# gaozhihan/PreDiff

Hardware: AMD Instinct MI355X
Metric: denoising_steps_per_sec (higher is better)
Workload: dtype bf16; 1 GPU; SEVIR-LR 7->6 x128x128 (latent 13x16x16, C 256/512, depth [4,4], axial), DDIM-50 eta=0, no knowledge alignment (BASELINE.json configs[1]); trajectories_per_gpu=64, global_trajectories=64, sampler=ddim50, hip_graph=True, lanes=2, trajectories_per_launch=32, parallelism=ensemble-shard x1

## Files before the change

### prediff_amd/csrc/conv3d_halo.hip

```cpp
#include <algorithm>
#include "common.h"
#include "igemm_epilogue.h"

namespace PD_NS {

#define BLDS16(rsrc, ldsptr, voff, soff) \
  __builtin_amdgcn_raw_ptr_buffer_load_lds((rsrc), (__attribute__((address_space(3))) void*)(ldsptr), 16, (voff), (soff), 0, 0)
#define PD_OOB 0xffffff00u
#define VMCNT(n) asm volatile("s_waitcnt vmcnt(" #n ")" ::: "memory")
#define PHASE_SYNC()                   \
  __builtin_amdgcn_sched_barrier(0);   \
  __builtin_amdgcn_s_barrier();        \
  __builtin_amdgcn_sched_barrier(0)

namespace {
constexpr int FW = 16;
constexpr int HW = FW + 2;
constexpr int HROWS = HW * HW;
constexpr int PLROWS = 336;
constexpr int PLANE = PLROWS * 16;
constexpr int HALO = 8 * PLANE;
constexpr int NPIECE = HALO / 1024;
constexpr int WHT = 128 * 128;
constexpr int WBUF = 2 * WHT;
// ... 88 lines not shown
  const bool dense = (p.debug_flags & 8) != 0;
  const int kt_lo = (dense || L) ? 0 : max(0, 1 - ot), kt_hi = (dense || L) ? 2 : min(2, p.Ti - ot);
  const int ngroups = (p.debug_flags & 1) ? 0 : kchunks * (kt_hi - kt_lo + 1);
  const uint32_t frame_b = (uint32_t)(L ? FW1 * FW1 : FW * FW) * (uint32_t)p.lda * 2u;
  uint32_t vm_all = 0;
  if constexpr (L == 1) {
    int o = (4 * tm) % p.To;
    for (int f = 0; f < 4; ++f) {
      if (4 * tm + f < p.B * p.To)
        for (int kt = 0; kt < 3; ++kt)
          if ((unsigned)(o - 1 + kt) < (unsigned)p.Ti) vm_all |= 1u << (4 * kt + f);
      if (++o == p.To) o = 0;
    }
  }
  const uint32_t w_tap_b = (uint32_t)p.w_tap_stride * 2u;

  int h_c = 0, h_kt = kt_lo, w_c = 0, w_kt = kt_lo;
  uint32_t w_off = (uint32_t)(kt_lo * 9) * w_tap_b;
  int h_soff = 0;
  uint32_t h_mask = 0, h_back = 0;
  char* const h_dst = smem + wave * 1024;
  char* const w_dst = smem + W_OFF + wave * 1024;
  auto next_halo = [&]() {
    if constexpr (L == 0) {
      const int it = ot - 1 + h_kt;
      const bool ok = (unsigned)it < (unsigned)p.Ti;
      h_soff = __builtin_amdgcn_readfirstlane(ok ? (int)((uint32_t)(tm - 1 + h_kt) * frame_b + (uint32_t)h_c * 128u) : 0);
      h_mask = ok ? 0u : PD_OOB;
    } else {
      const int fin = 4 * tm - 1 + h_kt, fb = max(fin, 0);
      h_soff = __builtin_amdgcn_readfirstlane((int)((uint32_t)fb * frame_b + (uint32_t)h_c * 128u));
      h_back = (uint32_t)(fb - fin) * frame_b;
      h_mask = (vm_all >> (4 * h_kt)) & 15u;
    }
    if (++h_kt > kt_hi) { h_kt = kt_lo; ++h_c; }
  };
  auto issue_h = [&](int n, int buf) {
    uint32_t v;
    if constexpr (L == 0) v = hoff[n] | h_mask;
    else v = ((h_mask >> (hoff[n] & 7u)) & 1u) ? (hoff[n] & ~7u) - h_back : PD_OOB;
    BLDS16(rA, h_dst + buf * HALO + n * 8192, v, h_soff);
  };
  auto next_w_group = [&]() {
    if (++w_kt > kt_hi) { w_kt = kt_lo; ++w_c; }
    w_off = (uint32_t)(w_kt * 9) * w_tap_b + (uint32_t)w_c * 128u;
  };
  auto issue_w = [&](int buf) {
    const int so = __builtin_amdgcn_readfirstlane((int)w_off);
    char* dst = w_dst + buf * WBUF;
    BLDS16(rW, dst, woff[0][0], so);
    BLDS16(rW, dst + 64 * 128, woff[0][1], so);
    BLDS16(rW, dst + WHT, woff[1][0], so);
    BLDS16(rW, dst + WHT + 64 * 128, woff[1][1], so);
    w_off += w_tap_b;
  };

  f32x4 acc[8][4];
#pragma unroll
  for (int i = 0; i < 8; ++i)
#pragma unroll
    for (int j = 0; j < 4; ++j)
#pragma unroll
      for (int r = 0; r < 4; ++r) acc[i][j][r] = 0.f;

  const int l16 = lane & 15, lg = lane >> 4;
  const int swz = (l16 >> 1) & 7;
  const int a_rd = (L ? wr * WROW1 + (l16 >> 3) * FPAIR1 + (l16 & 7) : wr * (8 * HW) + l16) * 16 + lg * PLANE;
  const int b_rd = W_OFF + (wc >> 1) * WHT + ((wc & 1) * 64 + l16) * 128;

  if (ngroups > 0) {
    next_halo();
    if (wave < NEXTRA) issue_h(5, 0);
#pragma unroll
    for (int n = 0; n < 5; ++n) issue_h(n, 0);
    issue_w(0);
    issue_w(1);
    VMCNT(4);
  }
  __builtin_amdgcn_s_barrier();
  if (wr == 1) __builtin_amdgcn_s_barrier();
  __builtin_amdgcn_sched_barrier(0);

  FragH a[4], b0[2], b1[2];
#define LOAD_B(f, base) \
  (f).v[0] = *(const op8*)((base) + ((lg ^ swz) * 16)); (f).v[1] = *(const op8*)((base) + (((4 + lg) ^ swz) * 16))
#define LOAD_A(f, base) \
  (f).v[0] = *(const op8*)(base); (f).v[1] = *(const op8*)((base) + 4 * PLANE)
#define QUAD16(R0, C0, bfrag)                                                                               \
  _Pragma("unroll") for (int ks = 0; ks < 2; ++ks)                                                          \
    _Pragma("unroll") for (int i = 0; i < 4; ++i)                                                           \
      _Pragma("unroll") for (int c = 0; c < 2; ++c)                                                         \
        acc[(R0) + i][(C0) + c] = mfma_16x16x32(a[i].v[ks], bfrag[c].v[ks], acc[(R0) + i][(C0) + c]);

  int wcur = 0;
  auto group = [&](auto has_next_t, int g) {
    constexpr bool has_next = decltype(has_next_t)::value;
    const int hnxt = (g & 1) ^ 1;
    const char* sA = smem + (g & 1) * HALO + a_rd;
    if (has_next) next_halo();
#pragma unroll
    for (int j = 0; j < 9; ++j) {
      const int shift = ((j / 3) * PITCH + (j % 3)) * 16;
      const char* sB = smem + wcur * WBUF + b_rd;
#pragma unroll
      for (int c = 0; c < 2; ++c) { LOAD_B(b0[c], sB + c * (16 * 128)); }
#pragma unroll
      for (int i = 0; i < 4; ++i) { LOAD_A(a[i], sA + shift + i * (PITCH * 16)); }
#pragma unroll
      for (int c = 0; c < 2; ++c) { LOAD_B(b1[c], sB + (2 + c) * (16 * 128)); }
      if (j >= 1 && j <= 5 && has_next) {
        if (j == 1 && wave < NEXTRA) issue_h(5, hnxt);
        issue_h(j - 1, hnxt);
      }
      PHASE_SYNC();
      __builtin_amdgcn_s_setprio(1);
      QUAD16(0, 0, b0)
      QUAD16(0, 2, b1)
      __builtin_amdgcn_s_setprio(0);
      PHASE_SYNC();
#pragma unroll
      for (int i = 0; i < 4; ++i) { LOAD_A(a[i], sA + shift + (4 + i) * (PITCH * 16)); }
      if (j <= 6 || has_next) {
        if (j == 7) next_w_group();
        issue_w(wcur);
        if (j >= 1 && j <= 5 && has_next) {
          VMCNT(5);
        } else {
          VMCNT(4);
        }
      } else {
        VMCNT(0);
      }
      PHASE_SYNC();
      __builtin_amdgcn_s_setprio(1);
      QUAD16(4, 2, b1)
      QUAD16(4, 0, b0)
      __builtin_amdgcn_s_setprio(0);
      PHASE_SYNC();
      wcur ^= 1;
    }
  };
  for (int g = 0; g + 1 < ngroups; ++g) group(std::true_type{}, g);
  if (ngroups > 0) group(std::false_type{}, ngroups - 1);
#undef QUAD16
#undef LOAD_A
#undef LOAD_B
  if (wr == 0) __builtin_amdgcn_s_barrier();
  if (p.debug_flags & 2) return;

  float* sC = (float*)smem + wave * (128 * 32);
  const int m_base = m0 + wr * 128;
  const int m_end = min(p.M, m_base + 128);
  const int c_row = L ? (lg >> 1) * 64 + (lg & 1) * 4 : 4 * lg;
#pragma unroll
  for (int js = 0; js < 2; ++js) {
    __syncthreads();
#pragma unroll
    for (int i = 0; i < 8; ++i)
#pragma unroll
      for (int c = 0; c < 2; ++c)
#pragma unroll
        for (int r = 0; r < 4; ++r) sC[(c_row + i * (L ? 8 : 16) + r) * 32 + c * 16 + l16] = acc[i][js * 2 + c][r];
    __syncthreads();
    igemm_epilogue<128, 32>(p, sC, lane, m_base, m_end, n0 + wc * 64 + js * 32, 0);
  }
#endif
}

bool pd_conv3d_halo_supported(const pd_igemm_args& a, int kind, int level) {
  if (kind != 2 || a.split || a.fp8 || a.w_fold > 0 || a.nbatch > 1) return false;
  if (a.KT != 3 || a.KH != 3 || a.KW != 3 || a.pt != 1 || a.ph != 1 || a.pw != 1) return false;
  if (a.st != 1 || a.sh != 1 || a.sw != 1 || a.ut != 1 || a.uh != 1 || a.uw != 1 || a.vT > 0 || a.vH > 0 || a.vW > 0) return false;
  const int fw = level ? FW1 : FW;
  return a.Hi == fw && a.Wi == fw && a.Ho == fw && a.Wo == fw && a.Ti == a.To;
}

template <int L>
static int launch_halo(const pd_igemm_args& a, hipStream_t s) {
  constexpr int LDS = Lay<L>::LDS;
  static bool attr_set_dev[PD_MAX_DEVICES];
  bool& attr_set = attr_set_dev[pd_cur_device()];
  if (!attr_set) {
    hipError_t e = hipFuncSetAttribute((const void*)conv3d_halo_kernel<L>, hipFuncAttributeMaxDynamicSharedMemorySize, LDS);
    if (e != hipSuccess) {
      pd_set_error("pd_igemm: hipFuncSetAttribute(%d) failed: %s", LDS, hipGetErrorString(e));
      return PD_ERR_LAUNCH;
    }
    attr_set = true;
  }
  const int tiles = ((a.M + 255) / 256) * ((a.N + 255) / 256);
  hipLaunchKernelGGL(conv3d_halo_kernel<L>, dim3(tiles, 1, 1), dim3(512), LDS, s, a);
  PD_CHECK_LAUNCH();
  return PD_OK;
}

int pd_conv3d_halo_launch(const pd_igemm_args& a, int level, hipStream_t s) { return level ? launch_halo<1>(a, s) : launch_halo<0>(a, s); }

}
```

### prediff_amd/csrc/igemm.hip

```cpp
#include <type_traits>
#include "common.h"
#include "igemm_epilogue.h"

namespace PD_NS {

__device__ __attribute__((aligned(64))) uint32_t g_pd_zero_page[32];

#ifndef PD_BIG_TILE_DEFAULT
#define PD_BIG_TILE_DEFAULT 1
#endif

#define BLDS16(rsrc, ldsptr, voff, soff) \
  __builtin_amdgcn_raw_ptr_buffer_load_lds((rsrc), (__attribute__((address_space(3))) void*)(ldsptr), 16, (voff), (soff), 0, 0)
#define PD_OOB 0xffffff00u

template <int N>
__device__ __forceinline__ void wait_vmcnt() {
  asm volatile("s_waitcnt vmcnt(%0)" ::"n"(N) : "memory");
}

template <int BM, int BN, int BK, int NS, bool SPLIT, int KIND, int OCC = 2, int ESLAB = 1>
__global__ void __launch_bounds__(256, OCC) igemm_kernel(const pd_igemm_args p) {
#if defined(__HIP_DEVICE_COMPILE__)
  constexpr int ROWB = BK * 2;
// ... 8 lines not shown
  constexpr int KSUB = BK / 32;
  extern __shared__ __attribute__((aligned(16))) char smem[];

  const int tid = threadIdx.x;
  const int lane = tid & 63;
  const int wave = __builtin_amdgcn_readfirstlane(tid >> 6);

  const int tiles_n = (p.N + BN - 1) / BN;
  const int tiles_m = (p.M + BM - 1) / BM;
  const int nt = tiles_m * tiles_n;
  int t;
  {
    const int bid = blockIdx.x, xcd = bid & 7, q = nt >> 3, r = nt & 7;
    t = (xcd < r ? xcd * (q + 1) : r * (q + 1) + (xcd - r) * q) + (bid >> 3);
  }
  const int m0 = (t / tiles_n) * BM;
  const int n0 = (t % tiles_n) * BN;
  const int bz = blockIdx.z;

  const auto rA = __builtin_amdgcn_make_buffer_rsrc((void*)(p.A + (int64_t)bz * p.a_batch_stride), 0, p.a_bytes, 0x00020000);
  const auto rW = __builtin_amdgcn_make_buffer_rsrc((void*)(p.W + (int64_t)bz * p.w_batch_stride), 0, p.w_bytes, 0x00020000);
  const auto rAlo = __builtin_amdgcn_make_buffer_rsrc((void*)((SPLIT ? p.A_lo : p.A) + (int64_t)bz * p.a_batch_stride), 0, p.a_bytes, 0x00020000);
  const auto rWlo = __builtin_amdgcn_make_buffer_rsrc((void*)((SPLIT ? p.W_lo : p.W) + (int64_t)bz * p.w_batch_stride), 0, p.w_bytes, 0x00020000);

  const int srow = tid / CPR;
  const int spos = tid % CPR;
  const int schunk = (CPR == 8) ? (spos ^ ((srow >> 1) & 7)) : (spos ^ ((srow >> 2) & 3));
  int vt0[AI], vh0[AI], vw0[AI];
  uint32_t abase[AI];
  uint32_t aoff[AI];
#pragma unroll
  for (int i = 0; i < AI; ++i) {
    const int m = m0 + i * RPI + srow;
    if (KIND == 0) {
      aoff[i] = m < p.M ? ((uint32_t)m * (uint32_t)p.lda + schunk * 8) * 2u : PD_OOB;
    } else {
      const int hw_o = p.Ho * p.Wo, thw_o = p.To * hw_o;
      const bool ok = m < p.M;
      const int mm = ok ? m : 0;
      const int b = mm / thw_o, r1 = mm - b * thw_o;
      const int ot = r1 / hw_o, r2 = r1 - ot * hw_o;
      const int oh = r2 / p.Wo, ow = r2 - oh * p.Wo;
      vt0[i] = ok ? ot * p.st - p.pt : -(1 << 20);
      vh0[i] = oh * p.sh - p.ph;
      vw0[i] = ow * p.sw - p.pw;
      abase[i] = (uint32_t)b * (uint32_t)(p.Ti * p.Hi * p.Wi);
    }
  }
  uint32_t woff[BI];
#pragma unroll
  for (int i = 0; i < BI; ++i) {
    const int n = n0 + i * RPI + srow;
    woff[i] = n < p.N ? ((uint32_t)n * (uint32_t)p.ldw + schunk * 8) * 2u : PD_OOB;
  }
  const int kchunks = p.Cin / BK;
  const int nk = (p.debug_flags & 1) ? 0 : p.taps * kchunks;
  const int vT = p.vT > 0 ? p.vT : p.Ti * p.ut, vH = p.vH > 0 ? p.vH : p.Hi * p.uh, vW = p.vW > 0 ? p.vW : p.Wi * p.uw;
  const int khw = p.KH * p.KW;

  auto set_tap = [&](int tap) {
    if (p.w_fold > 0 && tap >= p.w_fold) tap -= p.w_fold;
    const int kt = tap / khw, r = tap - kt * khw;
    const int kh = r / p.KW, kw = r - kh * p.KW;
#pragma unroll
    for (int i = 0; i < AI; ++i) {
      const int vt = vt0[i] + kt, vh = vh0[i] + kh, vw = vw0[i] + kw;
      const bool ok = (unsigned)vt < (unsigned)vT && (unsigned)vh < (unsigned)vH && (unsigned)vw < (unsigned)vW;
      const int it = p.ut == 2 ? vt >> 1 : vt, ih = p.uh == 2 ? vh >> 1 : vh, iw = p.uw == 2 ? vw >> 1 : vw;
      aoff[i] = ok ? ((abase[i] + (uint32_t)((it * p.Hi + ih) * p.Wi + iw)) * (uint32_t)p.lda + schunk * 8) * 2u : PD_OOB;
    }
  };

  auto issue = [&](int stage, int ks) {
    const int tap = ks / kchunks, kc = ks - tap * kchunks;
    if (KIND != 0 && kc == 0) set_tap(tap);
    char* sbase = smem + stage * STAGE;
    const int ka = kc * (BK * 2);
    const int kw = (int)(((int64_t)tap * p.w_tap_stride + kc * BK) * 2);
#pragma unroll
    for (int i = 0; i < AI; ++i) {
      char* dst = sbase + (i * 256 + wave * 64) * 16;
      BLDS16(rA, dst, aoff[i], ka);
      if (SPLIT) BLDS16(rAlo, dst + A_TILE, aoff[i], ka);
    }
#pragma unroll
    for (int i = 0; i < BI; ++i) {
      char* dst = sbase + A_TILE * NP + (i * 256 + wave * 64) * 16;
      BLDS16(rW, dst, woff[i], kw);
      if (SPLIT) BLDS16(rWlo, dst + B_TILE, woff[i], kw);
    }
  };

  constexpr int TM16 = BM / 32, TN16 = BN / 32;
  f32x4 acc[TM16][TN16];
#pragma unroll
  for (int i = 0; i < TM16; ++i)
#pragma unroll
    for (int j = 0; j < TN16; ++j)
#pragma unroll
      for (int r = 0; r < 4; ++r) acc[i][j][r] = 0.f;

  const int wr = wave >> 1, wc = wave & 1;
  const int l16 = lane & 15, lg = lane >> 4;
  const int swz = (CPR == 8) ? ((l16 >> 1) & 7) : ((l16 >> 2) & 3);
  const int a_row_b = (wr * (BM / 2) + l16) * ROWB;
  const int b_row_b = (wc * (BN / 2) + l16) * ROWB;

  constexpr int D = NS - 1;
#pragma unroll
  for (int s0 = 0; s0 < D; ++s0)
    if (s0 < nk) issue(s0, s0);
  int stage = 0;
  for (int ks = 0; ks < nk; ++ks) {
    const int younger = min(D - 1, nk - ks - 1);
    if (D >= 3 && younger == 2) wait_vmcnt<2 * LPS>();
    else if (D >= 2 && younger == 1) wait_vmcnt<LPS>();
    else wait_vmcnt<0>();
    __builtin_amdgcn_s_barrier();
    if (ks + D < nk) issue((stage + D) % NS, ks + D);
    const char* sA = smem + stage * STAGE;
    const char* sB = sA + A_TILE * NP;
#pragma unroll
    for (int kk = 0; kk < KSUB; ++kk) {
      const int pos = ((kk * 4 + lg) ^ swz) * 16;
      op8 a[TM16], b[TN16], al[TM16], bl[TN16];
#pragma unroll
      for (int i = 0; i < TM16; ++i) {
        a[i] = *(const op8*)(sA + a_row_b + i * 16 * ROWB + pos);
        if (SPLIT) al[i] = *(const op8*)(sA + A_TILE + a_row_b + i * 16 * ROWB + pos);
      }
#pragma unroll
      for (int j = 0; j < TN16; ++j) {
        b[j] = *(const op8*)(sB + b_row_b + j * 16 * ROWB + pos);
        if (SPLIT) bl[j] = *(const op8*)(sB + B_TILE + b_row_b + j * 16 * ROWB + pos);
      }
#pragma unroll
      for (int i = 0; i < TM16; ++i)
#pragma unroll
        for (int j = 0; j < TN16; ++j) {
          if (SPLIT) {
            acc[i][j] = mfma_16x16x32(al[i], b[j], acc[i][j]);
            acc[i][j] = mfma_16x16x32(a[i], bl[j], acc[i][j]);
          }
          acc[i][j] = mfma_16x16x32(a[i], b[j], acc[i][j]);
        }
    }
    stage = stage + 1 == NS ? 0 : stage + 1;
  }

  constexpr int WM = BM / 2, WN = BN / 2;
  constexpr int WNS = WN / ESLAB;
  constexpr int TNS = TN16 / ESLAB;
  float* sC = (float*)smem + wave * (WM * WNS);
#pragma unroll
  for (int js = 0; js < ESLAB; ++js) {
    __syncthreads();
#pragma unroll
    for (int i = 0; i < TM16; ++i)
#pragma unroll
      for (int j = 0; j < TNS; ++j)
#pragma unroll
        for (int r = 0; r < 4; ++r)
          sC[(i * 16 + 4 * lg + r) * WNS + j * 16 + l16] = acc[i][js * TNS + j][r];
    __syncthreads();
    igemm_epilogue<WM, WNS>(p, sC, lane, m0 + wr * WM, p.M, n0 + wc * WN + js * WNS, bz);
  }
#endif
}

template <int BM, int BN, int BK, int NS, bool SPLIT, int KIND, int OCC = 2, int ESLAB = 1>
static int launch_igemm(const pd_igemm_args& a, hipStream_t s) {
  constexpr int stage = (BM + BN) * BK * 2 * (SPLIT ? 2 : 1);
  constexpr int epi = 4 * (BM / 2) * (BN / 2) * 4 / ESLAB;
  constexpr int lds = NS * stage > epi ? NS * stage : epi;
  static bool attr_set_dev[PD_MAX_DEVICES];
  bool& attr_set = attr_set_dev[pd_cur_device()];
  if (!attr_set) {
    hipError_t e = hipFuncSetAttribute((const void*)igemm_kernel<BM, BN, BK, NS, SPLIT, KIND, OCC, ESLAB>,
                                       hipFuncAttributeMaxDynamicSharedMemorySize, lds);
    if (e != hipSuccess) {
      pd_set_error("pd_igemm: hipFuncSetAttribute(%d) failed: %s", lds, hipGetErrorString(e));
      return PD_ERR_LAUNCH;
    }
    attr_set = true;
  }
  const int tiles = ((a.M + BM - 1) / BM) * ((a.N + BN - 1) / BN);
  dim3 grid(tiles, 1, a.nbatch > 0 ? a.nbatch : 1);
  hipLaunchKernelGGL((igemm_kernel<BM, BN, BK, NS, SPLIT, KIND, OCC, ESLAB>), grid, dim3(256), lds, s, a);
  PD_CHECK_LAUNCH();
  return PD_OK;
}

template <bool SPLIT, int KIND>
static int dispatch_igemm(const pd_igemm_args& a, int tile, hipStream_t s) {
  switch (tile) {
    case 1: return launch_igemm<128, 128, 64, 2, SPLIT, KIND>(a, s);
    case 2: return launch_igemm<64, 64, 64, 2, SPLIT, KIND>(a, s);
    case 3: return launch_igemm<128, 128, 32, 4, SPLIT, KIND>(a, s);
    case 4: return launch_igemm<128, 128, 64, 3, SPLIT, KIND>(a, s);
    case 5: return launch_igemm<128, 128, 32, 2, SPLIT, KIND, (SPLIT ? 2 : 4), 2>(a, s);
    case 6: return launch_igemm<128, 128, 32, 3, SPLIT, KIND, (SPLIT ? 2 : 3), 2>(a, s);
    case 8: return launch_igemm<128, 64, 64, 2, SPLIT, KIND>(a, s);
    case 9: return launch_igemm<64, 128, 64, 2, SPLIT, KIND>(a, s);
    default: pd_set_error("pd_igemm: unknown tile config %d", tile); return PD_ERR_ARG;
  }
}

bool pd_igemm256_supported(const pd_igemm_args& a, int kind);
int pd_igemm256_launch(const pd_igemm_args& a, int kind, hipStream_t s);

int pd_igemm256_ksplit(const pd_igemm_args& a, int kind);
int pd_igemm256_launch_splitk(const pd_igemm_args& a, int kind, hipStream_t s);

bool pd_conv3d_halo_supported(const pd_igemm_args& a, int kind, int level);
int pd_conv3d_halo_launch(const pd_igemm_args& a, int level, hipStream_t s);

bool pd_igemm_operand_extents(pd_igemm_args& a) {
  const int eb = a.fp8 ? 1 : 2;
  const int64_t abytes = (int64_t)a.B * a.Ti * a.Hi * a.Wi * (int64_t)a.lda * eb;
  const int64_t wbytes = ((int64_t)(a.taps - 1) * a.w_tap_stride + (int64_t)a.N * a.ldw) * eb;
  if (abytes >= 0xfffffe00ll || wbytes >= 0xfffffe00ll) return false;
  a.a_bytes = (uint32_t)abytes;
  a.w_bytes = (uint32_t)wbytes;
  return true;
}
int pd_igemm_vec_epilogue(const pd_igemm_args& a) {
  const bool v4 = ((a.N & 3) == 0) && (!a.out_f32 || (a.ld_out & 3) == 0) && (!a.out_bf16 || (a.ld_outb & 3) == 0) &&
                  (!a.residual || (a.ld_res & 3) == 0) && (!a.rowvec || (a.ld_rowvec & 3) == 0) &&
                  (!a.mul || (a.ld_mul & 3) == 0) && (((uintptr_t)a.out_f32 | (uintptr_t)a.residual | (uintptr_t)a.rowvec |
                  (uintptr_t)a.mul) & 15) == 0 && (((uintptr_t)a.out_bf16 | (uintptr_t)a.out_bf16_lo) & 7) == 0 &&
                  ((a.out_batch_stride | a.outb_batch_stride | a.res_batch_stride) & 3) == 0;
  if (v4 && !a.out_f32 && a.out_bf16 && (a.N & 7) == 0 && (a.ld_outb & 7) == 0 && (a.outb_batch_stride & 7) == 0 &&
      (((uintptr_t)a.out_bf16 | (uintptr_t)a.out_bf16_lo) & 15) == 0)
    return 2;
  return v4 ? 1 : 0;
}

#if !PD_IS_F16
extern "C" int pd_f16_igemm(const pd_igemm_args*, pd_stream_t);
#endif

extern "C" int PD_ENTRY(igemm)(const pd_igemm_args* pa, pd_stream_t stream) {
  PD_CHECK_ARG(pa != nullptr, "pd_igemm: null args");
  PD_FORWARD_F16(pa->operand == PD_OPERAND_F16, pd_f16_igemm(pa, stream));
  pd_igemm_args a = *pa;
  PD_CHECK_ARG(!PD_IS_F16 || (!a.split && !a.fp8 && !a.out_bf16_lo), "pd_igemm: IEEE-half operands: no hi/lo split, no e4m3 operands");
  const int min_k_256 = a.min_k_256 > 0 ? a.min_k_256 : a.split ? 256 : 1024;
  PD_CHECK_ARG(a.A && a.W, "pd_igemm: A/W null");
  PD_CHECK_ARG(a.M > 0 && a.N > 0 && a.taps > 0, "pd_igemm: bad M/N/taps (%d,%d,%d)", a.M, a.N, a.taps);
  PD_CHECK_ARG(a.Cin > 0 && (a.Cin & 63) == 0, "pd_igemm: Cin=%d must be a positive multiple of 64 (zero padded)", a.Cin);
  PD_CHECK_ARG((a.lda & 7) == 0 && (a.ldw & 7) == 0, "pd_igemm: lda/ldw must be multiples of 8 (16 B rows)");
  PD_CHECK_ARG(a.w_fold >= 0 && (a.w_fold == 0 || (!a.split && !a.fp8 && a.taps == 2 * a.w_fold)),
               "pd_igemm: w_fold = %d needs taps = 2 w_fold (W_hi slabs then W_lo slabs), no hi/lo split, no e4m3 operands", a.w_fold);
  PD_CHECK_ARG((a.w_fold ? a.w_fold : a.taps) == a.KT * a.KH * a.KW, "pd_igemm: taps != KT*KH*KW");
  PD_CHECK_ARG((int64_t)a.B * a.To * a.Ho * a.Wo == a.M, "pd_igemm: M != B*To*Ho*Wo");
  PD_CHECK_ARG((a.ut == 1 || a.ut == 2) && (a.uh == 1 || a.uh == 2) && (a.uw == 1 || a.uw == 2), "pd_igemm: bad upsample");
  if (a.fp8) {
    PD_CHECK_ARG((a.Cin & 127) == 0 && (a.lda & 15) == 0 && (a.ldw & 15) == 0, "pd_igemm: fp8 operands need Cin %% 128 == 0 and lda/ldw %% 16 == 0");
    PD_CHECK_ARG(!a.split && a.nbatch <= 1, "pd_igemm: fp8 operands: no hi/lo split, no batch");
  }
  PD_CHECK_ARG(pd_igemm_operand_extents(a), "pd_igemm: operand larger than a 4 GiB buffer descriptor");
  PD_CHECK_ARG(!a.split || (a.A_lo && a.W_lo), "pd_igemm: split needs A_lo and W_lo");
  PD_CHECK_ARG(!a.rowvec || a.rows_per_sample > 0, "pd_igemm: rowvec needs rows_per_sample");
  PD_CHECK_ARG(a.out_f32 || a.out_bf16, "pd_igemm: no output");
  hipStream_t s = (hipStream_t)stream;
  a.vec_epilogue = pd_igemm_vec_epilogue(a);
  if (a.out_fp8_log2 > 0) {
    PD_CHECK_ARG(a.vec_epilogue == 2 && !a.out_bf16_lo && !a.split && a.out_fp8_log2 <= 16,
                 "pd_igemm: an e4m3 output needs the 8-column vector epilogue (out_bf16 only, N %% 8 == 0, ld_outb %% 8 == 0, 16 B aligned), no split");
  }
  int tile = a.tile;
  const bool pointwise = (a.taps == 1 || a.w_fold == 1) && a.st == 1 && a.sh == 1 && a.sw == 1 && a.pt == 0 && a.ph == 0 && a.pw == 0 && a.ut == 1 &&
                         a.uh == 1 && a.uw == 1 && a.Ti == a.To && a.Hi == a.Ho && a.Wi == a.Wo && a.vT <= 0 && a.vH <= 0 && a.vW <= 0;
  const int kind = pointwise ? 0 : ((a.KT == 1 && a.Ti == 1 && a.To == 1) ? 1 : 2);
  a.ksplit = 1;
#if !PD_IS_F16
  if (a.fp8) {
    if (!pd_igemm256_supported(a, kind) || kind == 1) {
      pd_set_error("pd_igemm: fp8 operands are built for row-wise linear layers and stride-1, un-upsampled Conv3d launches only");
      return PD_ERR_UNSUPPORTED;
    }
    const int ks = (a.tile == 0 && !a.disable_256 && a.out_fp8_log2 <= 0) ? pd_igemm256_ksplit(a, kind) : 0;
    if (ks >= 2) {
      a.ksplit = ks;
      return pd_igemm256_launch_splitk(a, kind, s);
    }
    return pd_igemm256_launch(a, kind, s);
  }
#endif
  if (tile == 0 && !a.disable_256) {
    const int ks = pd_igemm256_ksplit(a, kind);
    if (ks >= 2) {
      a.ksplit = ks;
      return pd_igemm256_launch_splitk(a, kind, s);
    }
  }
  if (tile == 0) {
    const int64_t t128 = (int64_t)((a.M + 127) / 128) * ((a.N + 127) / 128) * (a.nbatch > 0 ? a.nbatch : 1);
    tile = t128 >= 192 ? ((!a.split && (int64_t)a.taps * a.Cin <= 256) ? 5 : PD_BIG_TILE_DEFAULT) : 2;
    if (tile == PD_BIG_TILE_DEFAULT && !a.disable_256 && (int64_t)a.taps * a.Cin >= min_k_256 && pd_igemm256_supported(a, kind)) {
      const int64_t t256 = (int64_t)((a.M + 255) / 256) * ((a.N + 255) / 256) * (a.nbatch > 0 ? a.nbatch : 1);
      const int64_t ncu = pd_num_cus();
      const int64_t r128 = a.split ? (t128 + ncu - 1) / ncu : (t128 + 2 * ncu - 1) / (2 * ncu), r256 = (t256 + ncu - 1) / ncu;
      if (a.split ? r256 * 11 <= r128 * 5 : r256 * 33 <= r128 * 20) tile = 7;
      if (tile == 7 && !(a.debug_flags & 16))
        tile = pd_conv3d_halo_supported(a, kind, 0) ? 10 : pd_conv3d_halo_supported(a, kind, 1) ? 11 : 7;
    }
  }
  if (tile == 10 || tile == 11) {
    if (pd_conv3d_halo_supported(a, kind, tile - 10)) return pd_conv3d_halo_launch(a, tile - 10, s);
    tile = 7;
  }
  if (a.split && tile == 4) tile = 1;
  if (tile == 7) {
    if (pd_igemm256_supported(a, kind)) return pd_igemm256_launch(a, kind, s);
    tile = PD_BIG_TILE_DEFAULT;
  }
#if !PD_IS_F16
  if (a.split) {
// ... 12 lines not shown
```

### prediff_amd/csrc/igemm256.hip

```cpp
#include <algorithm>
#include "common.h"
#include "igemm_epilogue.h"

namespace PD_NS {

#define BLDS16(rsrc, ldsptr, voff, soff) \
  __builtin_amdgcn_raw_ptr_buffer_load_lds((rsrc), (__attribute__((address_space(3))) void*)(ldsptr), 16, (voff), (soff), 0, 0)
#define BLDS4(rsrc, ldsptr, voff, soff) \
  __builtin_amdgcn_raw_ptr_buffer_load_lds((rsrc), (__attribute__((address_space(3))) void*)(ldsptr), 4, (voff), (soff), 0, 0)
#define PD_OOB 0xffffff00u
#define VMCNT(n) asm volatile("s_waitcnt vmcnt(" #n ")" ::: "memory")
#define PHASE_SYNC()                   \
  __builtin_amdgcn_sched_barrier(0);   \
  __builtin_amdgcn_s_barrier();        \
  __builtin_amdgcn_sched_barrier(0)

typedef int i32x8 __attribute__((ext_vector_type(8)));
typedef int i32x4v __attribute__((ext_vector_type(4)));

namespace {
template <bool F8>
struct Frag256 {
  op8 v[2];
  __device__ __forceinline__ void load(const char* base, int lg, int swz) {
// ... 253 lines not shown
#pragma unroll
  for (int i = 0; i < RT; ++i)
#pragma unroll
    for (int j = 0; j < 4; ++j)
#pragma unroll
      for (int r = 0; r < 4; ++r) acc[i][j][r] = 0.f;

  const int l16 = lane & 15, lg = lane >> 4;
  const int swz = (l16 >> 1) & 7;
  const int a_rd = wr * HT + l16 * 128;
  const int b_rd = (2 + (wc >> 1)) * HT + ((wc & 1) * 64 + l16) * 128;

  if (nk > 0) {
    issue_a(0, 0);
    issue_a(1, 0);
    issue_s(0);
    next_a();
    issue_w(0);
    if (nk > 1) {
      issue_w(1);
      VMCNT(4);
    } else {
      VMCNT(0);
    }
  }
  __builtin_amdgcn_s_barrier();
  if (wr == 1) __builtin_amdgcn_s_barrier();
  __builtin_amdgcn_sched_barrier(0);

  Frag256<F8> a[4], b0[2], b1[2];
  [[maybe_unused]] int sa[4], sb0[2], sb1[2];
#define QUAD16(NR, R0, C0, bfrag, sbfrag)                                                                                 \
  if constexpr (F8) {                                                                                                     \
    _Pragma("unroll") for (int i = 0; i < (NR); ++i)                                                                      \
      _Pragma("unroll") for (int c = 0; c < 2; ++c)                                                                       \
        if constexpr (MX) acc[(R0) + i][(C0) + c] = mfma_mx(a[i], bfrag[c], sa[i], sbfrag[c], acc[(R0) + i][(C0) + c]);   \
        else acc[(R0) + i][(C0) + c] = mfma_f8(a[i], bfrag[c], acc[(R0) + i][(C0) + c]);                                  \
      \
     \
    _Pragma("unroll") for (int i = 0; i < (NR); ++i)                                                                      \
      _Pragma("unroll") for (int c = 0; c < 2; ++c) asm volatile("" : "+v"(acc[(R0) + i][(C0) + c]));                     \
  } else if constexpr (SP) {                                                                                              \
    _Pragma("unroll") for (int i = 0; i < (NR); ++i)                                                                      \
      _Pragma("unroll") for (int c = 0; c < 2; ++c) {                                                                     \
        acc[(R0) + i][(C0) + c] = mfma_16x16x32(a[i].v[1], bfrag[c].v[0], acc[(R0) + i][(C0) + c]);           \
        acc[(R0) + i][(C0) + c] = mfma_16x16x32(a[i].v[0], bfrag[c].v[1], acc[(R0) + i][(C0) + c]);           \
        acc[(R0) + i][(C0) + c] = mfma_16x16x32(a[i].v[0], bfrag[c].v[0], acc[(R0) + i][(C0) + c]);           \
      }                                                                                                                   \
  } else {                                                                                                                \
    _Pragma("unroll") for (int ks = 0; ks < 2; ++ks)                                                                      \
      _Pragma("unroll") for (int i = 0; i < (NR); ++i)                                                                    \
        _Pragma("unroll") for (int c = 0; c < 2; ++c)                                                                     \
          acc[(R0) + i][(C0) + c] = mfma_op16(a[i], bfrag[c], ks, acc[(R0) + i][(C0) + c]);                               \
  }
  for (int kt = 0; kt < nk; ++kt) {
    const int cur = kt & 1;
    const char* sA = smem + cur * KBUF + a_rd;
    const char* sB = smem + cur * KBUF + b_rd;
    const bool more1 = kt + 1 < nk, more2 = kt + 2 < nk;

    if constexpr (P2) {
#pragma unroll
      for (int c = 0; c < 2; ++c) b0[c].load(sB + c * (16 * 128), lg, swz);
#pragma unroll
      for (int i = 0; i < RA0; ++i) a[i].load(sA + i * (16 * 128), lg, swz);
#pragma unroll
      for (int c = 0; c < 2; ++c) b1[c].load(sB + (2 + c) * (16 * 128), lg, swz);
      if constexpr (MX) {
        const char* sS = smem + cur * SBUF;
#pragma unroll
        for (int c = 0; c < 2; ++c) {
          sb0[c] = *(const uint8_t*)(sS + sr.rd_b + c * 64);
          sb1[c] = *(const uint8_t*)(sS + sr.rd_b + (2 + c) * 64);
        }
#pragma unroll
        for (int i = 0; i < RA0; ++i) sa[i] = *(const uint8_t*)(sS + sr.rd_a + i * 64);
      }
      if (more1) { issue_a(0, cur ^ 1); issue_a(1, cur ^ 1); issue_s(cur ^ 1); next_a(); }
      PHASE_SYNC();
      __builtin_amdgcn_s_setprio(1);
      QUAD16(RA0, 0, 0, b0, sb0)
      QUAD16(RA0, 0, 2, b1, sb1)
      __builtin_amdgcn_s_setprio(0);
      PHASE_SYNC();
#pragma unroll
      for (int i = 0; i < RA1; ++i) a[i].load(sA + (RA0 + i) * (16 * 128), lg, swz);
      if constexpr (MX) {
#pragma unroll
        for (int i = 0; i < RA1; ++i) sa[i] = *(const uint8_t*)(smem + cur * SBUF + sr.rd_a + (RA0 + i) * 64);
      }
      if (more2) {
        issue_w(cur);
        VMCNT(4);
      } else {
        VMCNT(0);
      }
      PHASE_SYNC();
      __builtin_amdgcn_s_setprio(1);
      QUAD16(RA1, RA0, 2, b1, sb1)
      QUAD16(RA1, RA0, 0, b0, sb0)
      __builtin_amdgcn_s_setprio(0);
      PHASE_SYNC();
      continue;
    }
#pragma unroll
    for (int c = 0; c < 2; ++c) b0[c].load(sB + c * (16 * 128), lg, swz);
#pragma unroll
    for (int i = 0; i < RA0; ++i) a[i].load(sA + i * (16 * 128), lg, swz);
    if (more1) issue_a(0, cur ^ 1);
    PHASE_SYNC();
    __builtin_amdgcn_s_setprio(1);
    QUAD16(RA0, 0, 0, b0, sb0)
    __builtin_amdgcn_s_setprio(0);
    PHASE_SYNC();

#pragma unroll
    for (int c = 0; c < 2; ++c) b1[c].load(sB + (2 + c) * (16 * 128), lg, swz);
    if (more1) { issue_a(1, cur ^ 1); next_a(); }
    PHASE_SYNC();
    __builtin_amdgcn_s_setprio(1);
    QUAD16(RA0, 0, 2, b1, sb1)
    __builtin_amdgcn_s_setprio(0);
    PHASE_SYNC();

#pragma unroll
    for (int i = 0; i < RA1; ++i) a[i].load(sA + (RA0 + i) * (16 * 128), lg, swz);
    PHASE_SYNC();
    __builtin_amdgcn_s_setprio(1);
    QUAD16(RA1, RA0, 2, b1, sb1)
    __builtin_amdgcn_s_setprio(0);
    PHASE_SYNC();

    if (more2) {
      issue_w(cur);
      VMCNT(4);
    } else {
      VMCNT(0);
    }
    PHASE_SYNC();
    __builtin_amdgcn_s_setprio(1);
    QUAD16(RA1, RA0, 0, b0, sb0)
    __builtin_amdgcn_s_setprio(0);
    PHASE_SYNC();
  }
#undef QUAD16
  if (wr == 0) __builtin_amdgcn_s_barrier();
  if (p.debug_flags & 2) return;

  float* sC = (float*)smem + wave * (128 * 32);
  constexpr int SKIP1 = 16 * RT - ROW1 > 0 ? 16 * RT - ROW1 : 0;
  const int skip = wr == 1 ? SKIP1 : 0;
  const int m_base = m0 + wr * ROW1 + skip;
  const int m_end = min(p.M, m0 + (wr == 0 ? 16 * RT : BM));
#pragma unroll
  for (int js = 0; js < 2; ++js) {
    __syncthreads();
#pragma unroll
    for (int i = 0; i < RT; ++i)
#pragma unroll
      for (int c = 0; c < 2; ++c)
#pragma unroll
        for (int r = 0; r < 4; ++r) sC[(i * 16 + 4 * lg + r) * 32 + c * 16 + l16] = acc[i][js * 2 + c][r];
    __syncthreads();
    if (SK) {
      pd_igemm_args q = p;
      q.bias = nullptr; q.rowvec = nullptr; q.mul = nullptr; q.residual = nullptr; q.out_bf16 = nullptr; q.out_bf16_lo = nullptr;
      q.out_f32 = p.splitk_ws + (int64_t)kslice * p.M * p.N;
      q.ld_out = p.N; q.alpha = 1.f; q.act = 0; q.out_batch_stride = 0;
      q.vec_epilogue = (p.N & 3) == 0 ? 1 : 0;
      igemm_epilogue<128, 32>(q, sC + skip * 32, lane, m_base, m_end, n0 + wc * 64 + js * 32, 0);
    } else {
      igemm_epilogue<128, 32>(p, sC + skip * 32, lane, m_base, m_end, n0 + wc * 64 + js * 32, bz);
    }
  }
#endif
}



__global__ void __launch_bounds__(256) igemm_splitk_reduce_kernel(const pd_igemm_args p) {
  const int n4 = p.N >> 2;
  const int64_t total = (int64_t)p.M * n4;
  const int64_t slab = (int64_t)p.M * p.N;
  for (int64_t i = (int64_t)blockIdx.x * 256 + threadIdx.x; i < total; i += (int64_t)gridDim.x * 256) {
    const int m = (int)(i / n4), n = (int)(i - (int64_t)m * n4) * 4;
    const float* src = p.splitk_ws + (int64_t)m * p.N + n;
    float4 acc = *(const float4*)src;
    for (int k = 1; k < p.ksplit; ++k) {
      const float4 t = *(const float4*)(src + k * slab);
      acc.x += t.x; acc.y += t.y; acc.z += t.z; acc.w += t.w;
    }
    float v[4] = {acc.x, acc.y, acc.z, acc.w};
    if (p.vec_epilogue && !p.mul && p.act == 0 && ((uintptr_t)p.bias & 15) == 0) {
      float4 b4 = make_float4(0.f, 0.f, 0.f, 0.f), r4 = b4, s4 = b4;
      if (p.bias) b4 = *(const float4*)(p.bias + n);
      if (p.rowvec) r4 = *(const float4*)(p.rowvec + (int64_t)(m / p.rows_per_sample) * p.ld_rowvec + n);
      if (p.residual) s4 = *(const float4*)(p.residual + (int64_t)(p.res_period ? m % p.res_period : m) * p.ld_res + n);
      const float bb[4] = {b4.x, b4.y, b4.z, b4.w}, rr[4] = {r4.x, r4.y, r4.z, r4.w}, ss[4] = {s4.x, s4.y, s4.z, s4.w};
#pragma unroll
      for (int e = 0; e < 4; ++e) {
        v[e] = v[e] * p.alpha + bb[e];
        if (p.rowvec) v[e] += rr[e];
        if (p.residual) v[e] += ss[e];
      }
      if (p.out_f32) *(float4*)(p.out_f32 + (int64_t)m * p.ld_out + n) = make_float4(v[0], v[1], v[2], v[3]);
      if (p.out_bf16) {
#pragma unroll
        for (int e = 0; e < 4; ++e) {
          uint16_t h, l;
          f2bf_split(v[e], h, l);
          p.out_bf16[(int64_t)m * p.ld_outb + n + e] = p.out_bf16_lo ? h : (uint16_t)f2op(v[e]);
          if (p.out_bf16_lo) p.out_bf16_lo[(int64_t)m * p.ld_outb + n + e] = l;
        }
      }
      continue;
    }
#pragma unroll
    for (int e = 0; e < 4; ++e) v[e] = v[e] * p.alpha + (p.bias ? p.bias[n + e] : 0.f);
    if (p.rowvec) {
      const float* rv = p.rowvec + (int64_t)(m / p.rows_per_sample) * p.ld_rowvec + n;
#pragma unroll
      for (int e = 0; e < 4; ++e) v[e] += rv[e];
    }
    if (p.act != 0) {
#pragma unroll
      for (int e = 0; e < 4; ++e) v[e] = (p.out_bf16 && !p.out_bf16_lo && !p.out_f32) ? act_apply16(v[e], p.act) : act_apply(v[e], p.act);
    }
    if (p.mul) {
      const float* mu = p.mul + (int64_t)m * p.ld_mul + n;
#pragma unroll
      for (int e = 0; e < 4; ++e) v[e] *= mu[e];
    }
    if (p.residual) {
      const float* rs = p.residual + (int64_t)(p.res_period ? m % p.res_period : m) * p.ld_res + n;
#pragma unroll
      for (int e = 0; e < 4; ++e) v[e] += rs[e];
    }
    if (p.out_f32) {
      float* o = p.out_f32 + (int64_t)m * p.ld_out + n;
      if (p.vec_epilogue) *(float4*)o = make_float4(v[0], v[1], v[2], v[3]);
      else { o[0] = v[0]; o[1] = v[1]; o[2] = v[2]; o[3] = v[3]; }
    }
    if (p.out_bf16) {
#pragma unroll
      for (int e = 0; e < 4; ++e) {
        uint16_t h, l;
        f2bf_split(v[e], h, l);
        p.out_bf16[(int64_t)m * p.ld_outb + n + e] = p.out_bf16_lo ? h : (uint16_t)f2op(v[e]);
        if (p.out_bf16_lo) p.out_bf16_lo[(int64_t)m * p.ld_outb + n + e] = l;
      }
    }
  }
}

template <int KIND, bool F8 = false, bool WF = false>
static int launch256_splitk(const pd_igemm_args& a, hipStream_t s) {
  constexpr int lds = 2 * KBUF;
  static bool attr_set_dev[PD_MAX_DEVICES];
  bool& attr_set = attr_set_dev[pd_cur_device()];
  if (!attr_set) {
    hipError_t e = hipFuncSetAttribute((const void*)igemm256_kernel<KIND, 8, true, F8, false, true, WF>, hipFuncAttributeMaxDynamicSharedMemorySize, lds);
    if (e != hipSuccess) {
      pd_set_error("pd_igemm: hipFuncSetAttribute(%d) failed: %s", lds, hipGetErrorString(e));
      return PD_ERR_LAUNCH;
    }
    attr_set = true;
  }
  const int tiles = ((a.M + 255) / 256) * ((a.N + 255) / 256);
  hipLaunchKernelGGL((igemm256_kernel<KIND, 8, true, F8, false, true, WF>), dim3(tiles, a.ksplit, 1), dim3(512), lds, s, a);
  PD_CHECK_LAUNCH();
  const int64_t total = (int64_t)a.M * (a.N >> 2);
  const unsigned blocks = (unsigned)std::min<int64_t>((total + 255) / 256, 4096);
  hipLaunchKernelGGL(igemm_splitk_reduce_kernel, dim3(blocks), dim3(256), 0, s, a);
  PD_CHECK_LAUNCH();
  return PD_OK;
}

bool pd_igemm256_supported(const pd_igemm_args& a, int kind);

int pd_igemm256_ksplit(const pd_igemm_args& a, int kind) {
  const int max_tiles = a.splitk_max_tiles > 0 ? a.splitk_max_tiles : a.splitk_max_tiles < 0 ? 0 : 128;
  if (!a.splitk_ws || a.split || (a.N & 3) || (a.nbatch > 1) || !pd_igemm256_supported(a, kind)) return 0;
  const int64_t tiles = (int64_t)((a.M + 255) / 256) * ((a.N + 255) / 256);
  const int nk = a.taps * (a.Cin >> (a.fp8 ? 7 : 6));
  if (tiles > max_tiles || nk < 32) return 0;
  int64_t ks = std::min<int64_t>(pd_num_cus() / tiles, nk / 8);
  ks = std::min<int64_t>(ks, a.splitk_ws_elems / ((int64_t)a.M * a.N));
  return ks >= 2 ? (int)ks : 0;
}

int pd_igemm256_launch_splitk(const pd_igemm_args& a, int kind, hipStream_t s) {
#if !PD_IS_F16
  if (a.fp8) return kind == 0 ? launch256_splitk<0, true>(a, s) : launch256_splitk<2, true>(a, s);
#endif
  if (a.w_fold > 0) return kind == 0 ? launch256_splitk<0, false, true>(a, s) : launch256_splitk<2, false, true>(a, s);
  return kind == 0 ? launch256_splitk<0>(a, s) : launch256_splitk<2>(a, s);
}

template <int KIND, int RT, bool F8 = false, bool SP = false, bool P2 = true, bool WF = false>
static int launch256(const pd_igemm_args& a, hipStream_t s) {
  constexpr int lds = 2 * KBUF;
  constexpr int BM = RT == 8 ? 256 : 16 * RT + 96;
  static bool attr_set_dev[PD_MAX_DEVICES];
  bool& attr_set = attr_set_dev[pd_cur_device()];
  if (!attr_set) {
    hipError_t e = hipFuncSetAttribute((const void*)igemm256_kernel<KIND, RT, false, F8, SP, P2, WF>, hipFuncAttributeMaxDynamicSharedMemorySize, lds);
    if (e != hipSuccess) {
      pd_set_error("pd_igemm: hipFuncSetAttribute(%d) failed: %s", lds, hipGetErrorString(e));
      return PD_ERR_LAUNCH;
    }
    attr_set = true;
  }
  const int tiles = ((a.M + BM - 1) / BM) * ((a.N + 255) / 256);
  dim3 grid(tiles, 1, a.nbatch > 0 ? a.nbatch : 1);
  hipLaunchKernelGGL((igemm256_kernel<KIND, RT, false, F8, SP, P2, WF>), grid, dim3(512), lds, s, a);
  PD_CHECK_LAUNCH();
  return PD_OK;
}

bool pd_igemm256_supported(const pd_igemm_args& a, int kind) {
  if (a.split) {
#if PD_IS_F16
    return false;
#else
    if (a.fp8 || a.nbatch > 1 || !a.A_lo || !a.W_lo) return false;
    const int64_t da = (const char*)a.A_lo - (const char*)a.A, dw = (const char*)a.W_lo - (const char*)a.W;
    if ((da < 0 ? -da : da) + (int64_t)a.a_bytes >= 0xfffffe00ll || (dw < 0 ? -dw : dw) + (int64_t)a.w_bytes >= 0xfffffe00ll) return false;
// ... 60 lines not shown
```

### prediff_amd/csrc/igemm_epilogue.h

```cpp
#pragma once
#include <type_traits>
#include "common.h"

template <int WM, int WNS, int CW, int ACT, int RV, int MU, int RS, int OF, int OB, int OL>
__device__ __forceinline__ void igemm_epilogue_rows(const pd_igemm_args& p, const float* sC, int lane, int m_base, int m_end, int n_base,
                                                    float* outf, pd_bf16* outb, pd_bf16* outbl, const float* res) {
  auto on = [](int tag, bool rt) { return tag == 2 ? rt : (tag == 1); };
  constexpr int LPR = WNS / CW;
  constexpr int RPP = 64 / LPR;
  const int c0 = (lane % LPR) * CW;
  const int n = n_base + c0;
  const bool vec = p.vec_epilogue && (n + CW - 1 < p.N);
  const bool has_rv = on(RV, p.rowvec != nullptr), has_mu = on(MU, p.mul != nullptr), has_rs = on(RS, res != nullptr);
  const bool has_of = on(OF, outf != nullptr), has_ob = on(OB, outb != nullptr), has_ol = on(OL, outbl != nullptr);
  const int act = ACT >= 0 ? ACT : ((p.debug_flags & 4) ? 0 : p.act);
  float bias_v[CW];
#pragma unroll
  for (int e = 0; e < CW; ++e) bias_v[e] = (p.bias && n + e < p.N) ? p.bias[n + e] : 0.f;
  if (n >= p.N || (p.debug_flags & 2)) return;
#pragma unroll 1
  for (int pass = 0; pass < WM / RPP; ++pass) {
    const int row = pass * RPP + lane / LPR;
    const int m = m_base + row;
    if (m >= m_end) continue;
    float v[CW];
#pragma unroll
    for (int q = 0; q < CW / 4; ++q) {
      const float4 a4 = *(const float4*)(sC + row * WNS + c0 + 4 * q);
      v[4 * q] = a4.x; v[4 * q + 1] = a4.y; v[4 * q + 2] = a4.z; v[4 * q + 3] = a4.w;
    }
    const float* rv = has_rv ? p.rowvec + (int64_t)(m / p.rows_per_sample) * p.ld_rowvec + n : nullptr;
    const float* mu = has_mu ? p.mul + (int64_t)m * p.ld_mul + n : nullptr;
    const float* rs = has_rs ? res + (int64_t)(p.res_period ? m % p.res_period : m) * p.ld_res + n : nullptr;
    if (vec) {
#pragma unroll
      for (int e = 0; e < CW; ++e) v[e] = v[e] * p.alpha + bias_v[e];
      if (has_rv) {
#pragma unroll
        for (int q = 0; q < CW / 4; ++q) { const float4 t4 = *(const float4*)(rv + 4 * q); v[4 * q] += t4.x; v[4 * q + 1] += t4.y; v[4 * q + 2] += t4.z; v[4 * q + 3] += t4.w; }
      }
      if (act != 0) {
        const bool only16 = (ACT == PD_ACT_GELU && OL == 0 && OF == 0) || (has_ob && !has_ol && !has_of);
#pragma unroll
        for (int e = 0; e < CW; ++e) v[e] = only16 ? act_apply16(v[e], act) : act_apply(v[e], act);
      }
      if (has_mu) {
#pragma unroll
        for (int q = 0; q < CW / 4; ++q) { const float4 t4 = *(const float4*)(mu + 4 * q); v[4 * q] *= t4.x; v[4 * q + 1] *= t4.y; v[4 * q + 2] *= t4.z; v[4 * q + 3] *= t4.w; }
      }
      if (has_rs) {
#pragma unroll
        for (int q = 0; q < CW / 4; ++q) { const float4 t4 = *(const float4*)(rs + 4 * q); v[4 * q] += t4.x; v[4 * q + 1] += t4.y; v[4 * q + 2] += t4.z; v[4 * q + 3] += t4.w; }
      }
      if (has_of) {
#pragma unroll
        for (int q = 0; q < CW / 4; ++q)
          *(float4*)(outf + (int64_t)m * p.ld_out + n + 4 * q) = make_float4(v[4 * q], v[4 * q + 1], v[4 * q + 2], v[4 * q + 3]);
      }
      if (CW == 8 && has_ob && p.out_fp8_log2 > 0) {
        const float f8s = __builtin_amdgcn_ldexpf(1.0f, p.out_fp8_log2);
        int w[2];
#pragma unroll
        for (int q = 0; q < 2; ++q) {
          float y[4];
#pragma unroll
          for (int k = 0; k < 4; ++k) y[k] = fminf(fmaxf(v[4 * q + k] * f8s, -448.f), 448.f);
          w[q] = __builtin_amdgcn_cvt_pk_fp8_f32(y[0], y[1], 0, false);
          w[q] = __builtin_amdgcn_cvt_pk_fp8_f32(y[2], y[3], w[q], true);
        }
        *(uint2*)((uint8_t*)outb + (int64_t)m * p.ld_outb + n) = make_uint2((uint32_t)w[0], (uint32_t)w[1]);
      } else if (has_ob) {
        uint32_t hi[CW / 2], lo[CW / 2];
#pragma unroll
        for (int e = 0; e < CW / 2; ++e) {
          if (has_ol) {
            uint16_t h0, l0, h1, l1;
            f2bf_split(v[2 * e], h0, l0);
            f2bf_split(v[2 * e + 1], h1, l1);
            hi[e] = h0 | ((uint32_t)h1 << 16);
            lo[e] = l0 | ((uint32_t)l1 << 16);
          } else {
            hi[e] = pack_op2(v[2 * e], v[2 * e + 1]);
          }
        }
        if constexpr (CW == 8) {
          *(uint4*)(outb + (int64_t)m * p.ld_outb + n) = make_uint4(hi[0], hi[1], hi[2], hi[3]);
          if (has_ol) *(uint4*)(outbl + (int64_t)m * p.ld_outb + n) = make_uint4(lo[0], lo[1], lo[2], lo[3]);
        } else {
          *(uint2*)(outb + (int64_t)m * p.ld_outb + n) = make_uint2(hi[0], hi[1]);
          if (has_ol) *(uint2*)(outbl + (int64_t)m * p.ld_outb + n) = make_uint2(lo[0], lo[1]);
        }
      }
    } else {
      for (int e = 0; e < CW; ++e) {
        if (n + e >= p.N) break;
        float x = v[e] * p.alpha + bias_v[e];
        if (rv) x += rv[e];
        x = (has_ob && !has_ol && !has_of) ? act_apply16(x, act) : act_apply(x, act);
        if (mu) x *= mu[e];
        if (rs) x += rs[e];
        if (has_of) outf[(int64_t)m * p.ld_out + n + e] = x;
        if (has_ob) {
          uint16_t h, l;
          f2bf_split(x, h, l);
          outb[(int64_t)m * p.ld_outb + n + e] = h;
          if (has_ol) outbl[(int64_t)m * p.ld_outb + n + e] = l;
        }
      }
    }
  }
}

template <int WM, int WNS>
__device__ __forceinline__ void igemm_epilogue(const pd_igemm_args& p, const float* sC, int lane, int m_base, int m_end, int n_base, int bz) {
  float* outf = p.out_f32 ? p.out_f32 + (int64_t)bz * p.out_batch_stride : nullptr;
  pd_bf16* outb = p.out_bf16 ? p.out_bf16 + (int64_t)bz * p.outb_batch_stride : nullptr;
  pd_bf16* outbl = p.out_bf16_lo ? p.out_bf16_lo + (int64_t)bz * p.outb_batch_stride : nullptr;
  const float* res = p.residual ? p.residual + (int64_t)bz * p.res_batch_stride : nullptr;
  const bool rvp = p.rowvec != nullptr, mup = p.mul != nullptr, rsp = res != nullptr, ofp = outf != nullptr, obp = outb != nullptr,
             olp = outbl != nullptr;
  const int actv = (p.debug_flags & 4) ? 0 : p.act;
  constexpr int GELU = PD_ACT_GELU;
  if (p.vec_epilogue == 2 && !rvp && !mup && !rsp && !ofp && obp && !olp && (actv == 0 || actv == GELU)) {
    if (actv == 0) igemm_epilogue_rows<WM, WNS, 8, 0, 0, 0, 0, 0, 1, 0>(p, sC, lane, m_base, m_end, n_base, outf, outb, outbl, res);
    else igemm_epilogue_rows<WM, WNS, 8, GELU, 0, 0, 0, 0, 1, 0>(p, sC, lane, m_base, m_end, n_base, outf, outb, outbl, res);
  } else if (p.vec_epilogue && ofp && !obp && !mup && actv == 0 && (rsp != rvp)) {
    if (rsp) igemm_epilogue_rows<WM, WNS, 4, 0, 0, 0, 1, 1, 0, 0>(p, sC, lane, m_base, m_end, n_base, outf, outb, outbl, res);
    else igemm_epilogue_rows<WM, WNS, 4, 0, 1, 0, 0, 1, 0, 0>(p, sC, lane, m_base, m_end, n_base, outf, outb, outbl, res);
  } else if (p.vec_epilogue == 2) {
    igemm_epilogue_rows<WM, WNS, 8, -1, 2, 2, 2, 2, 2, 2>(p, sC, lane, m_base, m_end, n_base, outf, outb, outbl, res);
  } else {
    igemm_epilogue_rows<WM, WNS, 4, -1, 2, 2, 2, 2, 2, 2>(p, sC, lane, m_base, m_end, n_base, outf, outb, outbl, res);
  }
}
```

Before: 1614 steps/s.

## Pipeline f32 residual/rowvec epilogue loads and use wave-local LDS syncs

Adds a batched f32 epilogue path that double-buffers the global residual or row-vector loads in groups of R rows, so those loads overlap with LDS reads and stores instead of being issued one row at a time. A uniform-sample fast path loads the row vector once. Each wave uses only its own LDS slab, so it also replaces block-wide __syncthreads between the slab write and read with a wave-local lgkmcnt wait. The cost is more register pressure and more template variants. Relaxing the barrier is only correct if no other wave touches that slab.

Measured after the change: 1634 steps/s, median of 6. 1.3% higher.

```diff
diff --git a/prediff_amd/csrc/conv3d_halo.hip b/prediff_amd/csrc/conv3d_halo.hip
--- a/prediff_amd/csrc/conv3d_halo.hip
+++ b/prediff_amd/csrc/conv3d_halo.hip
@@ -264,18 +264,21 @@
   const int m_base = m0 + wr * 128;
   const int m_end = min(p.M, m_base + 128);
   const int c_row = L ? (lg >> 1) * 64 + (lg & 1) * 4 : 4 * lg;
-#pragma unroll
-  for (int js = 0; js < 2; ++js) {
-    __syncthreads();
+  auto slab = [&](auto jsc) {
+    constexpr int js = decltype(jsc)::value;
+    if (js == 0) __syncthreads();
+    else igemm_epilogue_wave_sync();
 #pragma unroll
     for (int i = 0; i < 8; ++i)
 #pragma unroll
       for (int c = 0; c < 2; ++c)
 #pragma unroll
         for (int r = 0; r < 4; ++r) sC[(c_row + i * (L ? 8 : 16) + r) * 32 + c * 16 + l16] = acc[i][js * 2 + c][r];
-    __syncthreads();
+    igemm_epilogue_wave_sync();
     igemm_epilogue<128, 32>(p, sC, lane, m_base, m_end, n0 + wc * 64 + js * 32, 0);
-  }
+  };
+  slab(std::integral_constant<int, 0>{});
+  slab(std::integral_constant<int, 1>{});
 #endif
 }
 
diff --git a/prediff_amd/csrc/igemm.hip b/prediff_amd/csrc/igemm.hip
--- a/prediff_amd/csrc/igemm.hip
+++ b/prediff_amd/csrc/igemm.hip
@@ -184,9 +184,11 @@
   constexpr int WNS = WN / ESLAB;
   constexpr int TNS = TN16 / ESLAB;
   float* sC = (float*)smem + wave * (WM * WNS);
-#pragma unroll
-  for (int js = 0; js < ESLAB; ++js) {
-    __syncthreads();
+  static_assert(ESLAB == 1 || ESLAB == 2, "one call per slab below");
+  auto slab = [&](auto jsc) {
+    constexpr int js = decltype(jsc)::value;
+    if (js == 0) __syncthreads();
+    else igemm_epilogue_wave_sync();
 #pragma unroll
     for (int i = 0; i < TM16; ++i)
 #pragma unroll
@@ -194,9 +196,11 @@
 #pragma unroll
         for (int r = 0; r < 4; ++r)
           sC[(i * 16 + 4 * lg + r) * WNS + j * 16 + l16] = acc[i][js * TNS + j][r];
-    __syncthreads();
-    igemm_epilogue<WM, WNS>(p, sC, lane, m0 + wr * WM, p.M, n0 + wc * WN + js * WNS, bz);
-  }
+    igemm_epilogue_wave_sync();
+    igemm_epilogue<WM, WNS, 4>(p, sC, lane, m0 + wr * WM, p.M, n0 + wc * WN + js * WNS, bz);
+  };
+  slab(std::integral_constant<int, 0>{});
+  if constexpr (ESLAB > 1) slab(std::integral_constant<int, 1>{});
 #endif
 }
 
diff --git a/prediff_amd/csrc/igemm256.hip b/prediff_amd/csrc/igemm256.hip
--- a/prediff_amd/csrc/igemm256.hip
+++ b/prediff_amd/csrc/igemm256.hip
@@ -429,27 +429,30 @@
   const int skip = wr == 1 ? SKIP1 : 0;
   const int m_base = m0 + wr * ROW1 + skip;
   const int m_end = min(p.M, m0 + (wr == 0 ? 16 * RT : BM));
-#pragma unroll
-  for (int js = 0; js < 2; ++js) {
-    __syncthreads();
+  auto slab = [&](auto jsc) {
+    constexpr int js = decltype(jsc)::value;
+    if (js == 0) __syncthreads();
+    else igemm_epilogue_wave_sync();
 #pragma unroll
     for (int i = 0; i < RT; ++i)
 #pragma unroll
       for (int c = 0; c < 2; ++c)
 #pragma unroll
         for (int r = 0; r < 4; ++r) sC[(i * 16 + 4 * lg + r) * 32 + c * 16 + l16] = acc[i][js * 2 + c][r];
-    __syncthreads();
+    igemm_epilogue_wave_sync();
     if (SK) {
       pd_igemm_args q = p;
       q.bias = nullptr; q.rowvec = nullptr; q.mul = nullptr; q.residual = nullptr; q.out_bf16 = nullptr; q.out_bf16_lo = nullptr;
       q.out_f32 = p.splitk_ws + (int64_t)kslice * p.M * p.N;
       q.ld_out = p.N; q.alpha = 1.f; q.act = 0; q.out_batch_stride = 0;
       q.vec_epilogue = (p.N & 3) == 0 ? 1 : 0;
-      igemm_epilogue<128, 32>(q, sC + skip * 32, lane, m_base, m_end, n0 + wc * 64 + js * 32, 0);
+      igemm_epilogue<128, 32, (SKIP1 > 0 ? 0 : PD_EPI_R)>(q, sC + skip * 32, lane, m_base, m_end, n0 + wc * 64 + js * 32, 0);
     } else {
-      igemm_epilogue<128, 32>(p, sC + skip * 32, lane, m_base, m_end, n0 + wc * 64 + js * 32, bz);
-    }
-  }
+      igemm_epilogue<128, 32, (SKIP1 > 0 ? 0 : PD_EPI_R)>(p, sC + skip * 32, lane, m_base, m_end, n0 + wc * 64 + js * 32, bz);
+    }
+  };
+  slab(std::integral_constant<int, 0>{});
+  slab(std::integral_constant<int, 1>{});
 #endif
 }
 
diff --git a/prediff_amd/csrc/igemm_epilogue.h b/prediff_amd/csrc/igemm_epilogue.h
--- a/prediff_amd/csrc/igemm_epilogue.h
+++ b/prediff_amd/csrc/igemm_epilogue.h
@@ -111,7 +111,89 @@
   }
 }
 
-template <int WM, int WNS>
+#ifndef PD_EPI_R
+#define PD_EPI_R 4
+#endif
+template <int WM, int WNS, int RV, int RS, int R>
+__device__ __forceinline__ void igemm_epilogue_rows_f32(const pd_igemm_args& p, const float* sC, int lane, int m_base, int m_end, int n_base,
+                                                        float* outf, const float* res) {
+  static_assert(RV + RS == 1, "one global operand: the per-sample row vector or the residual");
+  constexpr int LPR = WNS / 4;
+  constexpr int RPP = 64 / LPR;
+  constexpr int NP = WM / RPP;
+  static_assert(NP % R == 0 && 3 * R < 63, "whole batches; loads + stores in flight fit the vmcnt field");
+  constexpr int NB = NP / R;
+  if (m_base >= m_end) return;
+  const int c0 = (lane % LPR) * 4;
+  const int row0 = lane / LPR;
+  const int n = n_base + c0;
+  const int m_last = m_end - 1;
+  float bias_v[4];
+#pragma unroll
+  for (int e = 0; e < 4; ++e) bias_v[e] = p.bias ? p.bias[n + e] : 0.f;
+  const float alpha = p.alpha;
+  auto run = [&](auto uni, auto full) {
+    constexpr bool UNI = decltype(uni)::value;
+    constexpr bool FULL = decltype(full)::value;
+    float4 rv0 = make_float4(0.f, 0.f, 0.f, 0.f);
+    if (UNI) rv0 = *(const float4*)(p.rowvec + (int64_t)(m_base / p.rows_per_sample) * p.ld_rowvec + n);
+    auto issue = [&](int b, float4(&d)[R]) {
+      if (UNI) return;
+      int src[R];
+#pragma unroll
+      for (int r = 0; r < R; ++r) src[r] = FULL ? m_base + (b * R + r) * RPP + row0 : min(m_base + (b * R + r) * RPP + row0, m_last);
+      if (RS) {
+        if (p.res_period) {
+#pragma unroll
+          for (int r = 0; r < R; ++r) src[r] %= p.res_period;
+        }
+      } else {
+#pragma unroll
+        for (int r = 0; r < R; ++r) src[r] /= p.rows_per_sample;
+      }
+      const float* base = (RS ? res : p.rowvec) + n;
+      const int ld = RS ? p.ld_res : p.ld_rowvec;
+#pragma unroll
+      for (int r = 0; r < R; ++r) d[r] = *(const float4*)(base + (int64_t)src[r] * ld);
+    };
+    float4 g[2][R];
+    issue(0, g[0]);
+#pragma unroll
+    for (int b = 0; b < NB; ++b) {
+      if (b + 1 < NB) issue(b + 1, g[(b + 1) & 1]);
+      float4 v[R];
+#pragma unroll
+      for (int r = 0; r < R; ++r) v[r] = *(const float4*)(sC + ((b * R + r) * RPP + row0) * WNS + c0);
+#pragma unroll
+      for (int r = 0; r < R; ++r) {
+        const float4 t4 = UNI ? rv0 : g[b & 1][r];
+        v[r].x = __builtin_fmaf(v[r].x, alpha, bias_v[0]) + t4.x;
+        v[r].y = __builtin_fmaf(v[r].y, alpha, bias_v[1]) + t4.y;
+        v[r].z = __builtin_fmaf(v[r].z, alpha, bias_v[2]) + t4.z;
+        v[r].w = __builtin_fmaf(v[r].w, alpha, bias_v[3]) + t4.w;
+        asm volatile("" : "+v"(v[r].x), "+v"(v[r].y), "+v"(v[r].z), "+v"(v[r].w));
+      }
+#pragma unroll
+      for (int r = 0; r < R; ++r) {
+        const int m = m_base + (b * R + r) * RPP + row0;
+        if (FULL || m < m_end) *(float4*)(outf + (int64_t)m * p.ld_out + n) = v[r];
+      }
+    }
+  };
+  const bool uni = RV && m_base / p.rows_per_sample == m_last / p.rows_per_sample;
+  const bool full = m_base + WM <= m_end;
+  if (RV && uni) {
+    if (full) run(std::true_type{}, std::true_type{});
+    else run(std::true_type{}, std::false_type{});
+  } else {
+    if (full) run(std::false_type{}, std::true_type{});
+    else run(std::false_type{}, std::false_type{});
+  }
+}
+
+__device__ __forceinline__ void igemm_epilogue_wave_sync() { asm volatile("s_waitcnt lgkmcnt(0)" ::: "memory"); }
+
+template <int WM, int WNS, int RMAX = PD_EPI_R>
 __device__ __forceinline__ void igemm_epilogue(const pd_igemm_args& p, const float* sC, int lane, int m_base, int m_end, int n_base, int bz) {
   float* outf = p.out_f32 ? p.out_f32 + (int64_t)bz * p.out_batch_stride : nullptr;
   pd_bf16* outb = p.out_bf16 ? p.out_bf16 + (int64_t)bz * p.outb_batch_stride : nullptr;
@@ -125,8 +207,16 @@
     if (actv == 0) igemm_epilogue_rows<WM, WNS, 8, 0, 0, 0, 0, 0, 1, 0>(p, sC, lane, m_base, m_end, n_base, outf, outb, outbl, res);
     else igemm_epilogue_rows<WM, WNS, 8, GELU, 0, 0, 0, 0, 1, 0>(p, sC, lane, m_base, m_end, n_base, outf, outb, outbl, res);
   } else if (p.vec_epilogue && ofp && !obp && !mup && actv == 0 && (rsp != rvp)) {
-    if (rsp) igemm_epilogue_rows<WM, WNS, 4, 0, 0, 0, 1, 1, 0, 0>(p, sC, lane, m_base, m_end, n_base, outf, outb, outbl, res);
-    else igemm_epilogue_rows<WM, WNS, 4, 0, 1, 0, 0, 1, 0, 0>(p, sC, lane, m_base, m_end, n_base, outf, outb, outbl, res);
+    constexpr int NP = WM / (64 / (WNS / 4));
+    constexpr int R = RMAX == 0 ? 1 : RMAX < NP ? RMAX : NP;
+    const bool serial = RMAX == 0 || (p.debug_flags & 32) || n_base + (lane % (WNS / 4)) * 4 + 3 >= p.N;
+    if (rsp) {
+      if (serial) igemm_epilogue_rows<WM, WNS, 4, 0, 0, 0, 1, 1, 0, 0>(p, sC, lane, m_base, m_end, n_base, outf, outb, outbl, res);
+      else if (!(p.debug_flags & 2)) igemm_epilogue_rows_f32<WM, WNS, 0, 1, R>(p, sC, lane, m_base, m_end, n_base, outf, res);
+    } else {
+      if (serial) igemm_epilogue_rows<WM, WNS, 4, 0, 1, 0, 0, 1, 0, 0>(p, sC, lane, m_base, m_end, n_base, outf, outb, outbl, res);
+      else if (!(p.debug_flags & 2)) igemm_epilogue_rows_f32<WM, WNS, 1, 0, R>(p, sC, lane, m_base, m_end, n_base, outf, res);
+    }
   } else if (p.vec_epilogue == 2) {
     igemm_epilogue_rows<WM, WNS, 8, -1, 2, 2, 2, 2, 2, 2>(p, sC, lane, m_base, m_end, n_base, outf, outb, outbl, res);
   } else {
```
